# netocg/vae-decode-hdr

Measured on NVIDIA B200. Metric: flux_vae_hdr_decode_megapixels_per_s, higher is better.
Workload: dtype fp16

## Files before the change

vae_decode_hdr_b200/csrc/api.cu:

```cuda
#include <stdarg.h>
#include <string.h>

#include <algorithm>
#include <functional>
#include <map>
#include <string>
#include <vector>

#include "engine.cuh"

namespace hdrvae {

static thread_local std::string g_last_error;
long long g_launch_count = 0;
void set_error(const char* fmt, ...) {
  char buf[1024];
  va_list ap;
  va_start(ap, fmt);
  vsnprintf(buf, sizeof buf, fmt, ap);
  va_end(ap);
  g_last_error = buf;
}

bool g_prof_on = false;
// ... 274 lines not shown
static bool nin_is_fused(hdrvae_ctx* ctx, const ResW& rw, int H, int W) {
  static int on = -1;
  if (on < 0) { const char* e = getenv("HDRVAE_FUSE_NIN"); on = (e && atoi(e) == 0) ? 0 : 1; }
  ConvIO probe;
  return on && rw.has_nin && !ctx->high && rw.nin_x16.w[0] != nullptr && conv_takes_slab(rw.c2, probe, H, W, ctx->conv_impl);
}

static bool x_is_16bit(hdrvae_ctx* ctx) {
  static int on = -1;
  if (on < 0) { const char* e = getenv("HDRVAE_X16"); on = (e && atoi(e) == 0) ? 0 : 1; }
  static int nin_on = -1;
  if (nin_on < 0) { const char* e = getenv("HDRVAE_FUSE_NIN"); nin_on = (e && atoi(e) == 0) ? 0 : 1; }
  return on && nin_on && !ctx->high && ctx->op_dtype == DT_F16 && ctx->conv_impl == HDRVAE_CONV_TCGEN05 && h_is_16bit(ctx);
}

static bool gn_is_fused(hdrvae_ctx* ctx, const PackedConv& pc, const ConvIO& io, int x_dtype, int H, int W) {
  static int on = -1;
  if (on < 0) {
    const char* e = getenv("HDRVAE_FUSE_GN");
    const char* g = getenv("HDRVAE_CTA_GROUP");
    on = ((e && atoi(e) == 0) || (g && atoi(g) == 1)) ? 0 : 1;
  }
  return on && x_is_16bit(ctx) && x_dtype == DT_F16 && pc.w_dtype == DT_F16 && pc.kmul == 1 && !pc.upsample && pc.ks == 3 &&
         pc.cout_pad >= 256 && pc.cin_pad % 64 == 0 && ctx->cta_group != 1 && io.x2 == nullptr && io.y_dtype == DT_F16 &&
         io.stats != nullptr && conv_takes_slab(pc, io, H, W, ctx->conv_impl);
}

static bool attention_fused_enabled(hdrvae_ctx* ctx) {
  static int on = -1;
  if (on < 0) { const char* e = getenv("HDRVAE_ATTN_FUSED"); on = (e && atoi(e) == 0) ? 0 : 1; }
// ... 71 lines not shown
      p.k_per_tap = ks; p.ntaps = 1;
      p.b = v; p.b_row_stride = Tp; p.b_rows = 512; p.n_cols = 512; p.b_img_k_stride = ks;
      p.out = part; p.out_dtype = DT_F32;
      p.out_px_stride = 512; p.out_row_stride = 0; p.out_img_stride = (long long)rows * 512;
      p.sy = p.sx = 1; p.alpha = 1.0f;
      p.tw_log2 = 7; p.TW = 128; p.TH = 1; p.tiles_x = (rows + 127) / 128; p.tiles_y = 1;
      p.cta_group = ctx->cta_group;
      if (impl == HDRVAE_CONV_DIRECT) HDRVAE_TRY(launch_gemm_direct(p, s));
      else HDRVAE_TRY(launch_gemm_tc(p, ctx->num_sms, s));
      HDRVAE_TRY(launch_attn_reduce_splits(part, inv, o_rows, dt, rows, 512, splits, s));
    }
  }
  return 0;
}

static int run_phase_a(hdrvae_ctx* ctx, const void* feat, int B, int H, int W, int pad, float* conv8, void* epi, cudaStream_t s) {
  static int tc_on = -1;
  if (tc_on < 0) { const char* e = getenv("HDRVAE_TC_CONVOUT"); tc_on = (e && atoi(e) == 0) ? 0 : 1; }
  const long long img_stride = (long long)(H + 2 * pad) * W * 128;
  if (ctx->high)
    return launch_epilogue_phase_a(feat, DT_F32, B, H, W, ctx->conv_out_w, ctx->conv_out_b, nullptr, epi, s, 0, img_stride);
  const uint16_t* interior = reinterpret_cast<const uint16_t*>(feat) + (size_t)pad * W * 128;
  if (tc_on && ctx->op_dtype == DT_F16 && ctx->conv_impl == HDRVAE_CONV_TCGEN05 && ctx->conv_out_tc.w[0] != nullptr) {
    ConvIO io; io.x = feat; io.x_pad = pad; io.y = conv8; io.y_dtype = DT_F32; io.y_channels = 8; io.n_store = 8;
    HDRVAE_TRY(run_conv(ctx, ctx->conv_out_tc, io, B, H, W, HDRVAE_CONV_TCGEN05, s));
    return launch_epilogue_phase_a_pre(interior, ctx->op_dtype, B, H, W, conv8, ctx->conv_out_b, nullptr, epi, s, img_stride);
  }
  return launch_epilogue_phase_a(interior, ctx->op_dtype, B, H, W, ctx->conv_out_w, ctx->conv_out_b, nullptr, epi, s, pad, img_stride);
}

static int run_attention_high(hdrvae_ctx* ctx, const Plan& pl, uint8_t* ws, const uint16_t* t3, uint16_t* o3, cudaStream_t s) {
  const int impl = ctx->conv_impl, T = pl.T, Tp = pl.Tp;
  float* f32 = reinterpret_cast<float*>(ws + pl.off_f32);
  uint16_t* q3 = reinterpret_cast<uint16_t*>(ws + pl.off_qk);
  uint16_t* k3 = q3 + (size_t)Tp * 1536;
  uint16_t* vt3 = reinterpret_cast<uint16_t*>(ws + pl.off_vt);
  float* S = reinterpret_cast<float*>(ws + pl.off_s);
  uint16_t* P3 = reinterpret_cast<uint16_t*>(ws + pl.off_p);
// ... 138 lines not shown
  hdrvae_rows* rows;
  cudaStream_t s;
  int B;
  int pad;
  void* lat;
  float* x;
  float* hbuf;
  void* t;
  void* xa16;
  void* xb16;
  void* gn;
  int gn_chunks;
  int* pending;
  int x_dt, h_dt;
  float x_scale, h_scale;
};

static Decoder make_decoder(hdrvae_ctx* ctx, hdrvae_rows* rows, cudaStream_t s, int B, int* pending) {
  Decoder d;
  memset(&d, 0, sizeof d);
  d.ctx = ctx; d.rows = rows; d.s = s; d.B = B; d.pad = rows != nullptr ? 1 : 0; d.pending = pending;
  const bool x16 = x_is_16bit(ctx), h16 = h_is_16bit(ctx);
  d.x_dt = x16 ? ctx->op_dtype : DT_F32; d.x_scale = x16 ? kRawOperandScale : 1.f;
  d.h_dt = h16 ? ctx->op_dtype : DT_F32; d.h_scale = h16 ? kRawOperandScale : 1.f;
  return d;
}

static int step(Decoder& d, std::function<int(cudaStream_t)> fn) {
  if (d.rows == nullptr) return fn(d.s);
  hdrvae_rows::Op op; op.exchange = false; op.fn = std::move(fn); memset(&op.ex, 0, sizeof op.ex);
// ... 117 lines not shown
  ConvIO sc; sc.x = d.xb16; sc.y = d.hbuf; sc.alpha = 1.0f / kRawOperandScale;
  HDRVAE_TRY(conv(d, rw.nin, sc, H, W, kNoStats));
  io.y = d.hbuf; io.residual = d.hbuf;
  HDRVAE_TRY(conv(d, rw.c2, io, H, W));
  std::swap(d.x, d.hbuf);
  return 0;
}

static int decode_to_attention(Decoder& d, int H, int W) {
  ConvIO io; io.x = d.lat; io.y = d.x; io.y_dtype = d.x_dt; io.y_scale = d.x_scale;
  HDRVAE_TRY(conv(d, d.ctx->conv_in, io, H, W, d.x_dt != DT_F32 ? kZeroHalos : 0));
  HDRVAE_TRY(decode_res(d, d.ctx->mid1, H, W));
  return norm(d, d.x, d.x_dt, d.x_scale, d.ctx->attn_norm, false, H, W);
}

static int decode_from_attention(Decoder& d, const void* o, int H, int W) {
  hdrvae_ctx* ctx = d.ctx;
  const bool x16 = d.x_dt != DT_F32;
  {
    ConvIO io; io.x = o; io.y = d.x; io.residual = d.x;
    io.y_dtype = d.x_dt; io.y_scale = d.x_scale; io.res_dtype = d.x_dt; io.res_scale = 1.f / d.x_scale;
    HDRVAE_TRY(conv(d, ctx->proj_out, io, H, W, kDenseInput));
  }
  HDRVAE_TRY(decode_res(d, ctx->mid2, H, W));
  for (int lvl = 3; lvl >= 0; --lvl) {
    for (int i = 0; i < 3; ++i) HDRVAE_TRY(decode_res(d, ctx->up[lvl][i], H, W));
    if (lvl != 0) {
      ConvIO io; io.x = d.xa16; io.y = d.hbuf; io.alpha = 1.0f / kRawOperandScale;
      if (x16) { io.x = d.x; io.y_dtype = d.x_dt; io.y_scale = d.x_scale; }
      else if (lvl <= 2) { io.y2 = d.xb16; io.y2_dtype = ctx->op_dtype; io.y2_scale = kRawOperandScale; }
      HDRVAE_TRY(conv(d, ctx->upsample[lvl], io, H, W, x16 ? kZeroHalos : 0));
      std::swap(d.x, d.hbuf);
      H *= 2; W *= 2;
    }
  }
  return norm(d, d.x, d.x_dt, d.x_scale, ctx->norm_out, true, H, W, ctx->high ? DT_F32 : -1);
}

static int attend_dense(Decoder& d, const Plan& pl, uint8_t* ws, const void** o_out) {
  hdrvae_ctx* ctx = d.ctx;
  const int B = d.B, impl = ctx->conv_impl, dt = ctx->op_dtype;
  cudaStream_t s = d.s;
  void* qk = ws + pl.off_qk;
  void* vt = ws + pl.off_vt;
  void* o = ws + pl.off_o;
  *o_out = o;
  if (ctx->high) {
    ProfScope prof("attention (high precision, GEMM form)", 4.0 * B * (double)pl.T * pl.T * 512 * 3, 0.0, s);
    for (int b = 0; b < B; ++b)
      HDRVAE_TRY(run_attention_high(ctx, pl, ws, reinterpret_cast<const uint16_t*>(d.t) + (size_t)b * pl.T * 1536,
// ... 6 lines not shown
    for (int b = 0; b < B; ++b) {
      const uint16_t* tb = reinterpret_cast<const uint16_t*>(d.t) + (size_t)b * pl.T * 512;
      HDRVAE_TRY(run_gemm(ctx, dt, tb, 512, pl.T, 512, ctx->qk.w[0], 512, 1024, 1024,
                          reinterpret_cast<uint16_t*>(qk) + (size_t)b * pl.Tp * 1024, 1024, dt, ctx->qk.bias, false, 1.0f,
                          nullptr, impl, s));
      HDRVAE_TRY(run_gemm(ctx, dt, ctx->vproj.w[0], 512, 512, 512, tb, 512, pl.T, pl.Tp,
                          reinterpret_cast<uint16_t*>(vt) + (size_t)b * 512 * pl.Tp, pl.Tp, dt, ctx->vproj.bias, true, 1.0f,
                          nullptr, impl, s));
    }
  }
  ProfScope prof("attention core (QK^T, softmax, PV)", 4.0 * B * (double)pl.T * pl.T * 512, 10.0 * B * (double)pl.T * pl.Tp, s);
  return run_attention_core(ctx, pl, ws, qk, vt, o, 1.0f, d.hbuf, (size_t)B * pl.T * 64 * 256 * 4, s);
}

static int run_decoder(hdrvae_ctx* ctx, const float* latent, const Plan& pl, uint8_t* ws, void** features,
                       cudaStream_t s) {
  HDRVAE_REQUIRE(ctx->loaded, "hdrvae: weights not loaded");
  const int B = pl.B, H = pl.h, W = pl.w;
  int pending = 0;
  Decoder d = make_decoder(ctx, nullptr, s, B, &pending);
  d.lat = ws + pl.off_lat;
  d.x = reinterpret_cast<float*>(ws + pl.off_x);
  d.hbuf = reinterpret_cast<float*>(ws + pl.off_h);
  d.t = ws + pl.off_t;
  d.xa16 = ws + pl.off_x16;
  d.xb16 = ws + pl.off_x16b;
  d.gn = ws + pl.off_gn;
  d.gn_chunks = pl.gn_chunks;
  HDRVAE_TRY(gn_scratch_reset(d.gn, B, pl.gn_chunks, s));
  if (ctx->high) {
    float* latf = reinterpret_cast<float*>(ws + pl.off_f32) + (size_t)pl.Tp * 1536;
    HDRVAE_TRY(launch_latent_to_nhwc(latent, latf, DT_F32, B, ctx->c_z, ctx->c_lat, ctx->pq_w, ctx->pq_b, H * W, 64, s));
    HDRVAE_TRY(launch_split3(latf, 64, d.lat, 192, (long long)B * H * W, 64, 1.f, 0, s));
  } else {
    HDRVAE_TRY(launch_latent_to_nhwc(latent, d.lat, ctx->op_dtype, B, ctx->c_z, ctx->c_lat, ctx->pq_w, ctx->pq_b, H * W, 64, s));
  }
  HDRVAE_TRY(decode_to_attention(d, H, W));
  const void* o = nullptr;
  HDRVAE_TRY(attend_dense(d, pl, ws, &o));
  HDRVAE_TRY(decode_from_attention(d, o, H, W));
  *features = d.t;
  return 0;
}

static void attend_rows(Decoder& d, int W, const void** o_out) {
  hdrvae_rows* st = d.rows;
  hdrvae_ctx* ctx = d.ctx;
  const RowsPlan& pl = st->pl;
  uint8_t* ws = st->ws;
  const int rank = st->rank, dt = ctx->op_dtype;
  uint16_t* qk = reinterpret_cast<uint16_t*>(ws + pl.off_qk);
  uint16_t* vb = reinterpret_cast<uint16_t*>(ws + pl.off_v);
  uint16_t* vt = reinterpret_cast<uint16_t*>(ws + pl.off_vt);
  uint16_t* o = reinterpret_cast<uint16_t*>(ws + pl.off_o);
  *o_out = o;
  const uint16_t* tl = reinterpret_cast<const uint16_t*>(d.t) + (size_t)W * 512;
// ... 331 lines not shown
  HDRVAE_CUDA_OK(cudaGraphLaunch(exec, s));
  return 0;
}

int hdrvae_decode_begin(hdrvae_ctx* ctx, const float* latent, int B, int h, int w, void* workspace, size_t ws_bytes,
                        void** raw_stats_dev, void* stream) {
  HDRVAE_REQUIRE(ctx != nullptr && latent != nullptr, "hdrvae_decode: null argument");
  HDRVAE_REQUIRE(B >= 1 && h >= 1 && w >= 1, "hdrvae_decode: empty latent batch [%d,%d,%d,%d]", B, ctx->c_lat, h, w);
  HDRVAE_CUDA_OK(cudaSetDevice(ctx->device));
  const Plan pl = make_plan(B, h, w, false, ctx->high, ctx->high || !attention_fused_enabled(ctx), ctx->c_lat);
  HDRVAE_TRY(check_ws(pl, workspace, ws_bytes));
  uint8_t* ws = reinterpret_cast<uint8_t*>(workspace);
  cudaStream_t s = reinterpret_cast<cudaStream_t>(stream);
  auto body = [&](const float* lat) -> int {
    void* feat = nullptr;
    HDRVAE_TRY(run_decoder(ctx, lat, pl, ws, &feat, s));
    ProfScope prof("epilogue phase A (conv_out, max-pool, stats)", 2.0 * B * 64.0 * h * w * 3 * 1152, B * 64.0 * h * w * (256 + 24), s);
    return run_phase_a(ctx, feat, B, 8 * h, 8 * w, 0, reinterpret_cast<float*>(ws + pl.off_h), ws + pl.off_epi, s);
  };
  if (graphs_enabled(ctx, s)) {
    float* lat_in = reinterpret_cast<float*>(ws + pl.off_lat_in);
    HDRVAE_CUDA_OK(cudaMemcpyAsync(lat_in, latent, (size_t)B * ctx->c_lat * pl.T * 4, cudaMemcpyDeviceToDevice, s));
    hdrvae_ctx::GraphEntry key{0, B, h, w, 0, ctx->conv_impl, ctx->cta_group, 0.f, 0.f, workspace, nullptr, 0};
    HDRVAE_TRY(run_segment(ctx, key, s, [&]() { return body(lat_in); }));
  } else {
    HDRVAE_TRY(body(latent));
  }
  if (raw_stats_dev != nullptr) *raw_stats_dev = epilogue_raw_stats_ptr(ws + pl.off_epi, B, 8 * h, 8 * w);
  return 0;
}

// ... 348 lines not shown
```

vae_decode_hdr_b200/csrc/common.cuh:

```cuda
#pragma once
#include <cuda.h>
#include <cuda_bf16.h>
#include <cuda_fp16.h>
#include <cuda_runtime.h>
#include <stdint.h>
#include <stdio.h>

#include <string>

namespace hdrvae {

void set_error(const char* fmt, ...);
extern long long g_launch_count;
#define HDRVAE_LAUNCHED() (++::hdrvae::g_launch_count)

#define HDRVAE_CUDA_OK(expr)                                                                  \
  do {                                                                                        \
    cudaError_t _e = (expr);                                                                  \
    if (_e != cudaSuccess) {                                                                  \
      ::hdrvae::set_error("%s:%d: %s -> %s", __FILE__, __LINE__, #expr, cudaGetErrorString(_e)); \
      return -1;                                                                              \
    }                                                                                         \
  } while (0)

// ... 118 lines not shown
  const float2 two = make_float2(2.f, 2.f);
  float2 r = make_float2(__int_as_float(0x7EF311C7 - __float_as_int(d.x)), __int_as_float(0x7EF311C7 - __float_as_int(d.y)));
  r = f2_mul(r, f2_fma(nd, r, two));
  r = f2_mul(r, f2_fma(nd, r, two));
  return f2_mul(v, r);
}
__device__ __forceinline__ float silu_nr(float v) {
  float e;
  asm("ex2.approx.ftz.f32 %0, %1;" : "=f"(e) : "f"(fminf(-v * 1.4426950408889634f, 80.f)));
  const float d = 1.f + e;
  float r = __int_as_float(0x7EF311C7 - __float_as_int(d));
  r = r * fmaf(-d, r, 2.f);
  r = r * fmaf(-d, r, 2.f);
  return v * r;
}
#endif

struct PerDeviceOnce {
  bool done[64] = {};
  bool first() {
    int d = 0;
    if (cudaGetDevice(&d) != cudaSuccess || d < 0 || d >= 64) return true;
    if (done[d]) return false;
    done[d] = true;
    return true;
  }
};

struct TensorMapPair {
  CUtensorMap a, b, a2, b2;
// ... 4 lines not shown
```

vae_decode_hdr_b200/csrc/engine.cuh:

```cuda
#pragma once
#include <string>
#include <vector>
#include <map>

#include "../../include/hdrvae.h"
#include "common.cuh"

namespace hdrvae {

int launch_gemm_tc(const GemmParams& p, int num_sms, cudaStream_t stream);
int launch_gemm_direct(const GemmParams& p, cudaStream_t s);
void choose_tile(int H, int W, GemmParams* p);
int launch_to_f32(const void* src, int dtype, float* dst, long long n, cudaStream_t s);
int launch_pack_weight(const float* w, void* out, int out_dtype, int cout, int cin, int ks, int ntaps, int cin_pad,
                       const int* tap_mask, float scale, cudaStream_t s, int split3 = 0);
int launch_add_vectors(const float* a, const float* b, float* c, int n, cudaStream_t s);
int launch_split3(const float* x, long long x_ld, void* out, long long out_ld, long long n, int C, float scale, int order,
                  cudaStream_t s);
int launch_latent_to_nhwc(const float* z, void* out, int out_dtype, int B, int C, int C_lat, const float* pq_w,
                          const float* pq_b, int HW, int cpad, cudaStream_t s);
int launch_latent_rows_to_nhwc(const float* z, void* out, int out_dtype, int C, int C_lat, const float* pq_w,
                               const float* pq_b, int h, int w, int y0, int rows, int cpad, cudaStream_t s);
int launch_softmax_rows(const float* s, void* p, int p_dtype, float* inv_sum, int n_rows, int n_valid, int n_pad,
                        long long s_ld, long long p_ld, cudaStream_t st);
// ... 16 lines not shown
                     float in_scale = 1.f);
size_t epilogue_scratch_bytes(int B, int H, int W);
void* epilogue_raw_stats_ptr(void* scratch, int B, int H, int W);
hdrvae_stats* epilogue_stats_dev_ptr(void* scratch, int B, int H, int W);
float* epilogue_post3_ptr(void* scratch, int B, int H, int W);
float* epilogue_pre3_ptr(void* scratch, int B, int H, int W);
int launch_epilogue_phase_a(const void* pre, int dtype, int B, int H, int W, const float* conv_w, const float* conv_b,
                            int* argmax3, void* scratch, cudaStream_t s, int y_pad = 0, long long img_stride = 0);
double* gn_sums_ptr(void* scratch, int B, int C, int max_chunks);
int launch_gn_reduce_partials(void* scratch, int B, int C, int max_chunks, int n_partials, cudaStream_t s);
int launch_gn_apply_from_sums(const void* x, int x_dtype, long long x_img_stride, void* y, int y_dtype, long long y_img_stride,
                              int B, int rows_px, int C, const float* gamma, const float* beta, bool silu, void* scratch,
                              int max_chunks, double count, cudaStream_t s, float in_scale = 1.f);
int launch_epilogue_phase_a_pre(const void* pre, int dtype, int B, int H, int W, const float* conv8, const float* conv_b,
                                int* argmax3, void* scratch, cudaStream_t s, long long img_stride);
int launch_split_hi_lo(const float* w, float* w8, int k, cudaStream_t s);
int launch_epilogue_phase_b(int B, int H, int W, int mode, float factor, float ev, float* out, hdrvae_stats* host_stats,
                            void* scratch, cudaStream_t s);
int attention_key_splits(int n_keys);
int launch_attention_fused(const void* q, long long q_ld, long long q_img_stride, int n_q, const void* k, long long k_ld,
                           long long k_img_stride, int k_rows, const void* vt, long long vt_ld, long long vt_img_stride,
                           int n_keys, void* o, long long o_img_stride, int n_img, int dt, float alpha, int cta_group,
                           int num_sms, float* part, float* ml, long long part_rows, cudaStream_t s);
int launch_raw_stats_merge(const hdrvae_raw_stats* blocks, int n, hdrvae_raw_stats* dst, cudaStream_t s);

constexpr int kRowsMaxRanks = 16;
struct RowsRawSlot { hdrvae_raw_stats s; unsigned char pad[32]; };
struct RowsMailbox {
  unsigned int arrived[64];
  unsigned int data[64];
// ... 139 lines not shown
```

vae_decode_hdr_b200/csrc/epilogue.cu:

```cuda
#include "../../include/hdrvae.h"
#include "common.cuh"

namespace hdrvae {

constexpr int kTileW = 64, kTileH = 16;
constexpr int kPxPerThread = 4;
constexpr int kHaloW = kTileW + 2, kHaloH = kTileH + 2;
constexpr int kRowPitch = 68;
constexpr int kTilePx = kHaloW * kHaloH;
constexpr int kChanStride = kRowPitch * kHaloH;
constexpr int kChunk = 16;
constexpr int kC = 128;
constexpr int kEpiThreads = (kTileW / kPxPerThread) * kTileH;

struct PartialA {
  float vmin[4];
  float vmax[4];
  double vsum[8];
};

struct PartialB {
  float omin, omax, imax, pad;
  unsigned long long hdr, neg, ihdr, pad2;
};
// ... 37 lines not shown
    const float2 b = __bfloat1622float2(*reinterpret_cast<const __nv_bfloat162*>(&r.y));
    return make_float4(a.x, a.y, b.x, b.y);
  }
};
template <> struct Cvt4<__half> {
  static __device__ __forceinline__ float4 cvt(const uint2& r) {
    const float2 a = __half22float2(*reinterpret_cast<const __half2*>(&r.x));
    const float2 b = __half22float2(*reinterpret_cast<const __half2*>(&r.y));
    return make_float4(a.x, a.y, b.x, b.y);
  }
};

__device__ __forceinline__ float warp_min(float v) { for (int o = 16; o; o >>= 1) v = fminf(v, __shfl_xor_sync(~0u, v, o)); return v; }
__device__ __forceinline__ float warp_max(float v) { for (int o = 16; o; o >>= 1) v = fmaxf(v, __shfl_xor_sync(~0u, v, o)); return v; }
__device__ __forceinline__ double warp_sum(double v) { for (int o = 16; o; o >>= 1) v += __shfl_xor_sync(~0u, v, o); return v; }

template <bool kArgmax>
__device__ __forceinline__ void maxpool_update(float v, int c, float& m, int& idx) {
  if (kArgmax) { if (v > m) { m = v; idx = c; } }
  else m = fmaxf(m, v);
}

template <typename T, bool kArgmax>
__global__ void __launch_bounds__(kEpiThreads, 2)
hdr_phase_a_kernel(const T* __restrict__ pre, const float* __restrict__ conv_w ,
                   const float* __restrict__ conv_b, int H, int W, float* __restrict__ post3,
                   float* __restrict__ pre3, int* __restrict__ argmax3, PartialA* __restrict__ partials, int y_pad,
                   long long img_stride) {
  extern __shared__ float sm[];
  float4* wsm = reinterpret_cast<float4*>(sm);
// ... 125 lines not shown
#pragma unroll
      for (int k = 0; k < 3; ++k) {
        const float cv = acc[q][k] + cb[k];
        const float sv = fminf(fmaxf(__fdiv_rn(__fadd_rn(cv, 1.0f), 2.0f), 0.f), 1.f);
        post3[o + k] = sv;
        pre3[o + k] = mx[q][k];
        if (kArgmax) argmax3[o + k] = am[q][k];
        cmin = fminf(cmin, cv); cmax = fmaxf(cmax, cv); csum += cv;
        pmin = fminf(pmin, sv); pmax = fmaxf(pmax, sv); psum += sv; psq += sv * sv;
        p3min = fminf(p3min, mx[q][k]); p3max = fmaxf(p3max, mx[q][k]);
        hl += mx[q][k] > 1.0f ? 1.f : 0.f;
      }
    }
  }

  __shared__ float rmin[4][8], rmax[4][8];
  __shared__ double rsum[8][8];
  const int warp = tid >> 5, lane = tid & 31;
  const float mins[4] = {warp_min(smin), warp_min(pmin), warp_min(cmin), warp_min(p3min)};
  const float maxs[4] = {warp_max(smax), warp_max(pmax), warp_max(cmax), warp_max(p3max)};
  const double sums[8] = {warp_sum((double)ssum), warp_sum((double)ssq), warp_sum((double)psum), warp_sum((double)psq),
                          warp_sum((double)csum), 0.0, warp_sum((double)nlive), warp_sum((double)hl)};
  if (lane == 0) {
    for (int k = 0; k < 4; ++k) { rmin[k][warp] = mins[k]; rmax[k][warp] = maxs[k]; }
    for (int k = 0; k < 8; ++k) rsum[k][warp] = sums[k];
  }
  __syncthreads();
  if (tid == 0) {
    PartialA pa;
    for (int k = 0; k < 4; ++k) {
      float a = rmin[k][0], b = rmax[k][0];
      for (int w2 = 1; w2 < 8; ++w2) { a = fminf(a, rmin[k][w2]); b = fmaxf(b, rmax[k][w2]); }
      pa.vmin[k] = a; pa.vmax[k] = b;
    }
    for (int k = 0; k < 8; ++k) {
      double a = 0.0;
      for (int w2 = 0; w2 < 8; ++w2) a += rsum[k][w2];
      pa.vsum[k] = a;
    }
    const int ix = min(kTileW, W - x0), iy = min(kTileH, H - y0);
    pa.vsum[5] = (double)ix * iy * kC;
    partials[(blockIdx.z * gridDim.y + blockIdx.y) * gridDim.x + blockIdx.x] = pa;
  }
}

template <typename T, bool kArgmax>
__global__ void __launch_bounds__(kEpiThreads)
hdr_phase_a_pre_kernel(const T* __restrict__ pre, const float4* __restrict__ conv8, const float* __restrict__ conv_b, int H,
                       int W, float* __restrict__ post3, float* __restrict__ pre3, int* __restrict__ argmax3,
                       PartialA* __restrict__ partials, long long img_stride) {
  const int img = blockIdx.z;
  const int x0 = blockIdx.x * kTileW, y0 = blockIdx.y * kTileH;
  const int tid = threadIdx.x, warp = tid >> 5, lane = tid & 31;
  const int sub = lane & 7;
  const int pq = lane >> 3;
  const T* img_base = pre + (long long)img * img_stride;
  const float cb[3] = {conv_b[0], conv_b[1], conv_b[2]};
  float smin = INFINITY, smax = -INFINITY, ssum = 0.f, ssq = 0.f;
// ... 68 lines not shown
      nlive += 3.f;
#pragma unroll
      for (int k = 0; k < 3; ++k) {
        const float cv = cvv[k];
        const float sv = fminf(fmaxf(__fdiv_rn(__fadd_rn(cv, 1.0f), 2.0f), 0.f), 1.f);
        post3[px * 3 + k] = sv;
        pre3[px * 3 + k] = mx[k];
        if (kArgmax) argmax3[px * 3 + k] = am[k];
        cmin = fminf(cmin, cv); cmax = fmaxf(cmax, cv); csum += cv;
        pmin = fminf(pmin, sv); pmax = fmaxf(pmax, sv); psum += sv; psq += sv * sv;
        p3min = fminf(p3min, mx[k]); p3max = fmaxf(p3max, mx[k]);
        hl += mx[k] > 1.0f ? 1.f : 0.f;
      }
    }
  }
  __shared__ float rmin[4][8], rmax[4][8];
  __shared__ double rsum[8][8];
  const float mins[4] = {warp_min(smin), warp_min(pmin), warp_min(cmin), warp_min(p3min)};
  const float maxs[4] = {warp_max(smax), warp_max(pmax), warp_max(cmax), warp_max(p3max)};
  const double sums[8] = {warp_sum((double)ssum), warp_sum((double)ssq), warp_sum((double)psum), warp_sum((double)psq),
                          warp_sum((double)csum), 0.0, warp_sum((double)nlive), warp_sum((double)hl)};
  if (lane == 0) {
    for (int k = 0; k < 4; ++k) { rmin[k][warp] = mins[k]; rmax[k][warp] = maxs[k]; }
    for (int k = 0; k < 8; ++k) rsum[k][warp] = sums[k];
  }
  __syncthreads();
  if (tid == 0) {
    PartialA pa;
    for (int k = 0; k < 4; ++k) {
      float a = rmin[k][0], b = rmax[k][0];
      for (int w2 = 1; w2 < 8; ++w2) { a = fminf(a, rmin[k][w2]); b = fmaxf(b, rmax[k][w2]); }
      pa.vmin[k] = a; pa.vmax[k] = b;
    }
    for (int k = 0; k < 8; ++k) {
      double a = 0.0;
      for (int w2 = 0; w2 < 8; ++w2) a += rsum[k][w2];
      pa.vsum[k] = a;
    }
    const int ix = min(kTileW, W - x0), iy = min(kTileH, H - y0);
    pa.vsum[5] = (double)ix * iy * kC;
    partials[(blockIdx.z * gridDim.y + blockIdx.y) * gridDim.x + blockIdx.x] = pa;
  }
}

__global__ void __launch_bounds__(256)
hdr_reduce_a_kernel(const PartialA* __restrict__ partials, int n, hdrvae_raw_stats* __restrict__ raw) {
  __shared__ float rmin[4][256], rmax[4][256];
  __shared__ double rsum[8][256];
  float mn[4], mx[4];
  double sm[8];
  for (int k = 0; k < 4; ++k) { mn[k] = INFINITY; mx[k] = -INFINITY; }
  for (int k = 0; k < 8; ++k) sm[k] = 0.0;
  for (int i = threadIdx.x; i < n; i += 256) {
    const PartialA pa = partials[i];
    for (int k = 0; k < 4; ++k) { mn[k] = fminf(mn[k], pa.vmin[k]); mx[k] = fmaxf(mx[k], pa.vmax[k]); }
    for (int k = 0; k < 8; ++k) sm[k] += pa.vsum[k];
  }
// ... 183 lines not shown
  st->hdr_pixels = (long long)hdr; st->negative_pixels = (long long)neg; st->intelligent_hdr_pixels = (long long)ihdr;
  st->accepted = (ihdr > 0 || imax > 1.1f) ? 1 : 0;
}

constexpr int kPhaseBBlocks = 148 * 8;

struct EpilogueScratch {
  float* post3; float* pre3; PartialA* pa; PartialB* pb; hdrvae_raw_stats* raw; HdrScalars* sc; hdrvae_stats* st;
};

static int n_blocks_a(int B, int H, int W) { return B * ceil_div(H, kTileH) * ceil_div(W, kTileW); }

size_t epilogue_scratch_bytes(int B, int H, int W) {
  size_t b = 0;
  b += align_up((size_t)B * H * W * 3 * sizeof(float), 256) * 2;
  b += align_up((size_t)n_blocks_a(B, H, W) * sizeof(PartialA), 256);
  b += align_up((size_t)kPhaseBBlocks * sizeof(PartialB), 256);
  b += 256 * 3;
  return b;
}

static EpilogueScratch carve(void* scratch, int B, int H, int W) {
  EpilogueScratch e;
  uint8_t* p = reinterpret_cast<uint8_t*>(scratch);
  const size_t img = align_up((size_t)B * H * W * 3 * sizeof(float), 256);
  e.post3 = reinterpret_cast<float*>(p); p += img;
  e.pre3 = reinterpret_cast<float*>(p); p += img;
  e.pa = reinterpret_cast<PartialA*>(p); p += align_up((size_t)n_blocks_a(B, H, W) * sizeof(PartialA), 256);
  e.pb = reinterpret_cast<PartialB*>(p); p += align_up((size_t)kPhaseBBlocks * sizeof(PartialB), 256);
  e.raw = reinterpret_cast<hdrvae_raw_stats*>(p); p += 256;
  e.sc = reinterpret_cast<HdrScalars*>(p); p += 256;
  e.st = reinterpret_cast<hdrvae_stats*>(p);
  return e;
}

void* epilogue_raw_stats_ptr(void* scratch, int B, int H, int W) { return carve(scratch, B, H, W).raw; }
hdrvae_stats* epilogue_stats_dev_ptr(void* scratch, int B, int H, int W) { return carve(scratch, B, H, W).st; }
float* epilogue_post3_ptr(void* scratch, int B, int H, int W) { return carve(scratch, B, H, W).post3; }
float* epilogue_pre3_ptr(void* scratch, int B, int H, int W) { return carve(scratch, B, H, W).pre3; }

template <typename T>
static void launch_phase_a(const void* pre, const float* conv_w, const float* conv_b, int H, int W, float* post3, float* pre3,
                           int* argmax3, PartialA* pa, dim3 grid, size_t smem, int y_pad, long long img_stride, cudaStream_t s) {
// ... 36 lines not shown
                                int* argmax3, void* scratch, cudaStream_t s, long long img_stride) {
  HDRVAE_REQUIRE(dtype == HDRVAE_F16 || dtype == HDRVAE_BF16, "epilogue (precomputed conv): 16-bit features only");
  if (img_stride == 0) img_stride = (long long)H * W * kC;
  EpilogueScratch e = carve(scratch, B, H, W);
  const dim3 grid(ceil_div(W, kTileW), ceil_div(H, kTileH), B);
  HDRVAE_REQUIRE(grid.y <= 65535 && grid.z <= 65535, "epilogue: image too large for the launch grid");
  const float4* c8 = reinterpret_cast<const float4*>(conv8);
#define HDRVAE_PA_PRE(T, AM) hdr_phase_a_pre_kernel<T, AM><<<grid, kEpiThreads, 0, s>>>(reinterpret_cast<const T*>(pre), c8, conv_b, \
                                                                                       H, W, e.post3, e.pre3, argmax3, e.pa, img_stride)
  if (dtype == HDRVAE_F16) { if (argmax3) HDRVAE_PA_PRE(__half, true); else HDRVAE_PA_PRE(__half, false); }
  else { if (argmax3) HDRVAE_PA_PRE(__nv_bfloat16, true); else HDRVAE_PA_PRE(__nv_bfloat16, false); }
#undef HDRVAE_PA_PRE
  HDRVAE_LAUNCHED();
  HDRVAE_CUDA_OK(cudaGetLastError());
  hdr_reduce_a_kernel<<<1, 256, 0, s>>>(e.pa, n_blocks_a(B, H, W), e.raw);
  HDRVAE_LAUNCHED();
  HDRVAE_CUDA_OK(cudaGetLastError());
  return 0;
}

int launch_epilogue_phase_b(int B, int H, int W, int mode, float factor, float ev, float* out, hdrvae_stats* host_stats,
                            void* scratch, cudaStream_t s) {
  EpilogueScratch e = carve(scratch, B, H, W);
  HDRVAE_REQUIRE(mode >= 0 && mode <= 3, "epilogue: bad mode %d", mode);
  hdr_scalars_kernel<<<1, 32, 0, s>>>(e.raw, e.sc, e.st);
  HDRVAE_LAUNCHED();
  HDRVAE_CUDA_OK(cudaGetLastError());
  const long long n = (long long)B * H * W * 3;
  int blocks = ceil_div(n, 256);
  if (blocks > kPhaseBBlocks) blocks = kPhaseBBlocks;
// ... 41 lines not shown
```

vae_decode_hdr_b200/csrc/groupnorm.cu:

```cuda
#include <type_traits>

#include "common.cuh"

namespace hdrvae {

constexpr int kGroups = 32;
constexpr int kGnThreads = 256;

template <typename T> struct Ld8;
template <> struct Ld8<float> {
  static __device__ __forceinline__ void ld(const float* p, float (&v)[8]) {
    const float4 a = __ldg(reinterpret_cast<const float4*>(p)), b = __ldg(reinterpret_cast<const float4*>(p) + 1);
    v[0] = a.x; v[1] = a.y; v[2] = a.z; v[3] = a.w; v[4] = b.x; v[5] = b.y; v[6] = b.z; v[7] = b.w;
  }
};
template <> struct Ld8<__nv_bfloat16> {
  static __device__ __forceinline__ void ld(const __nv_bfloat16* p, float (&v)[8]) {
    const uint4 r = __ldg(reinterpret_cast<const uint4*>(p));
    const __nv_bfloat162* h = reinterpret_cast<const __nv_bfloat162*>(&r);
#pragma unroll
    for (int e = 0; e < 4; ++e) { const float2 f = __bfloat1622float2(h[e]); v[2 * e] = f.x; v[2 * e + 1] = f.y; }
  }
};
template <> struct Ld8<__half> {
// ... 139 lines not shown
    const int g = c / cpg;
    const double mean = rs[0][g] / count;
    double var = rq[0][g] / count - mean * mean;
    if (var < 0.0) var = 0.0;
    const float rstd = (float)(1.0 / sqrt(var + (double)eps));
    const float a = gamma[c] * rstd;
    scale[(long long)img * C + c] = a;
    shift[(long long)img * C + c] = beta[c] - (float)mean * a;
  }
}
static int gn_slices(int n_chunks) {
  int sl = n_chunks / 32;
  return sl < 1 ? 1 : (sl > kGnSlices ? kGnSlices : sl);
}


template <int kExp> __device__ __forceinline__ float silu_sel(float v) {
  return kExp == 1 ? silu_mufu(v) : kExp == 2 ? silu_nr(v) : silu_f(v);
}

template <bool kSilu, int kExp>
__device__ __forceinline__ void norm_act8(float (&v)[8], const float (&a)[8], const float (&b)[8]) {
#pragma unroll
  for (int j = 0; j < 8; j += 2) {
    float2 t = f2_fma(make_float2(v[j], v[j + 1]), make_float2(a[j], a[j + 1]), make_float2(b[j], b[j + 1]));
    if (kSilu) {
      if (kExp == 2) t = silu_nr2(t);
      else t = make_float2(silu_sel<kExp>(t.x), silu_sel<kExp>(t.y));
    }
    v[j] = t.x; v[j + 1] = t.y;
  }
}

template <typename TIn, typename TOut, bool kSilu, int kMufu = 0>
__global__ void __launch_bounds__(kGnThreads)
gn_apply_kernel(const TIn* __restrict__ x, TOut* __restrict__ y, const float* __restrict__ scale,
                const float* __restrict__ shift, int HW, int C, int px_per_block, long long x_img_stride,
                long long y_img_stride, float in_scale) {
  extern __shared__ float tab[];
  const int img = blockIdx.y;
  for (int c = threadIdx.x; c < C; c += kGnThreads) {
    tab[c] = scale[(long long)img * C + c];
    tab[C + c] = shift[(long long)img * C + c];
  }
  __syncthreads();
  const int vpp = C >> 3;
  const int vi = threadIdx.x % vpp;
// ... 235 lines not shown
```

Baseline: 119.2.

## Fuse norm_out apply with pre-conv_out stats and max-pool in decoder tail

Adds a fused decoder tail. One kernel applies the final GroupNorm+SiLU, writes the fp16 activation, and also computes the pre-conv max-pool and stats. After the tensor-core conv_out, a separate post kernel computes the post-activation stats. Before, the normalized full-resolution 128-channel tensor was written by the GN apply and then re-read by epilogue phase A, so this removes one full pass over it at the cost of another kernel and a larger partials buffer.

```diff
diff --git a/vae_decode_hdr_b200/csrc/api.cu b/vae_decode_hdr_b200/csrc/api.cu
--- a/vae_decode_hdr_b200/csrc/api.cu
+++ b/vae_decode_hdr_b200/csrc/api.cu
@@ -312,6 +312,13 @@
   return on && nin_on && !ctx->high && ctx->op_dtype == DT_F16 && ctx->conv_impl == HDRVAE_CONV_TCGEN05 && h_is_16bit(ctx);
 }
 
+static bool conv_out_on_tc(hdrvae_ctx* ctx);
+static bool tail_is_fused(hdrvae_ctx* ctx) {
+  static int on = -1;
+  if (on < 0) { const char* e = getenv("HDRVAE_FUSED_TAIL"); on = (e && atoi(e) == 0) ? 0 : 1; }
+  return on && x_is_16bit(ctx) && conv_out_on_tc(ctx);
+}
+
 static bool gn_is_fused(hdrvae_ctx* ctx, const PackedConv& pc, const ConvIO& io, int x_dtype, int H, int W) {
   static int on = -1;
   if (on < 0) {
@@ -413,14 +420,18 @@
   return 0;
 }
 
-static int run_phase_a(hdrvae_ctx* ctx, const void* feat, int B, int H, int W, int pad, float* conv8, void* epi, cudaStream_t s) {
+static bool conv_out_on_tc(hdrvae_ctx* ctx) {
   static int tc_on = -1;
   if (tc_on < 0) { const char* e = getenv("HDRVAE_TC_CONVOUT"); tc_on = (e && atoi(e) == 0) ? 0 : 1; }
+  return tc_on && ctx->op_dtype == DT_F16 && ctx->conv_impl == HDRVAE_CONV_TCGEN05 && ctx->conv_out_tc.w[0] != nullptr;
+}
+
+static int run_phase_a(hdrvae_ctx* ctx, const void* feat, int B, int H, int W, int pad, float* conv8, void* epi, cudaStream_t s) {
   const long long img_stride = (long long)(H + 2 * pad) * W * 128;
   if (ctx->high)
     return launch_epilogue_phase_a(feat, DT_F32, B, H, W, ctx->conv_out_w, ctx->conv_out_b, nullptr, epi, s, 0, img_stride);
   const uint16_t* interior = reinterpret_cast<const uint16_t*>(feat) + (size_t)pad * W * 128;
-  if (tc_on && ctx->op_dtype == DT_F16 && ctx->conv_impl == HDRVAE_CONV_TCGEN05 && ctx->conv_out_tc.w[0] != nullptr) {
+  if (conv_out_on_tc(ctx)) {
     ConvIO io; io.x = feat; io.x_pad = pad; io.y = conv8; io.y_dtype = DT_F32; io.y_channels = 8; io.n_store = 8;
     HDRVAE_TRY(run_conv(ctx, ctx->conv_out_tc, io, B, H, W, HDRVAE_CONV_TCGEN05, s));
     return launch_epilogue_phase_a_pre(interior, ctx->op_dtype, B, H, W, conv8, ctx->conv_out_b, nullptr, epi, s, img_stride);
@@ -589,6 +600,7 @@
   int* pending;
   int x_dt, h_dt;
   float x_scale, h_scale;
+  void* epi;
 };
 
 static Decoder make_decoder(hdrvae_ctx* ctx, hdrvae_rows* rows, cudaStream_t s, int B, int* pending) {
@@ -736,6 +748,22 @@
   return norm(d, d.x, d.x_dt, d.x_scale, d.ctx->attn_norm, false, H, W);
 }
 
+static int fused_tail(Decoder& d, int H, int W) {
+  hdrvae_ctx* ctx = d.ctx;
+  const NormW& n = ctx->norm_out;
+  ProfScope prof("epilogue phase A (norm_out, conv_out, max-pool, stats)", 2.0 * d.B * H * W * 3 * 1152,
+                 d.B * (double)H * W * (256 + 256 + 12 + 256 + 32 + 32 + 12), d.s);
+  const int partials = *d.pending;
+  *d.pending = 0;
+  const float *scale = nullptr, *shift = nullptr;
+  HDRVAE_TRY(launch_gn_scale_shift(d.B, H * W, n.C, n.gamma, n.beta, d.gn, d.gn_chunks, partials, d.s, &scale, &shift));
+  HDRVAE_TRY(launch_epilogue_tail_pre(d.x, 1.f / d.x_scale, scale, shift, d.t, d.B, H, W, d.epi, d.s));
+  float* conv8 = d.hbuf;
+  ConvIO io; io.x = d.t; io.y = conv8; io.y_dtype = DT_F32; io.y_channels = 8; io.n_store = 8;
+  HDRVAE_TRY(run_conv(ctx, ctx->conv_out_tc, io, d.B, H, W, HDRVAE_CONV_TCGEN05, d.s));
+  return launch_epilogue_tail_post(conv8, ctx->conv_out_b, d.B, H, W, d.epi, d.s);
+}
+
 static int decode_from_attention(Decoder& d, const void* o, int H, int W) {
   hdrvae_ctx* ctx = d.ctx;
   const bool x16 = d.x_dt != DT_F32;
@@ -756,6 +784,7 @@
       H *= 2; W *= 2;
     }
   }
+  if (d.epi != nullptr) return fused_tail(d, H, W);
   return norm(d, d.x, d.x_dt, d.x_scale, ctx->norm_out, true, H, W, ctx->high ? DT_F32 : -1);
 }
 
@@ -792,7 +821,7 @@
 }
 
 static int run_decoder(hdrvae_ctx* ctx, const float* latent, const Plan& pl, uint8_t* ws, void** features,
-                       cudaStream_t s) {
+                       cudaStream_t s, void* epi = nullptr) {
   HDRVAE_REQUIRE(ctx->loaded, "hdrvae: weights not loaded");
   const int B = pl.B, H = pl.h, W = pl.w;
   int pending = 0;
@@ -805,6 +834,7 @@
   d.xb16 = ws + pl.off_x16b;
   d.gn = ws + pl.off_gn;
   d.gn_chunks = pl.gn_chunks;
+  if (epi != nullptr && tail_is_fused(ctx)) d.epi = epi;
   HDRVAE_TRY(gn_scratch_reset(d.gn, B, pl.gn_chunks, s));
   if (ctx->high) {
     float* latf = reinterpret_cast<float*>(ws + pl.off_f32) + (size_t)pl.Tp * 1536;
@@ -817,7 +847,7 @@
   const void* o = nullptr;
   HDRVAE_TRY(attend_dense(d, pl, ws, &o));
   HDRVAE_TRY(decode_from_attention(d, o, H, W));
-  *features = d.t;
+  *features = d.epi != nullptr ? nullptr : d.t;
   return 0;
 }
 
@@ -1179,7 +1209,8 @@
   cudaStream_t s = reinterpret_cast<cudaStream_t>(stream);
   auto body = [&](const float* lat) -> int {
     void* feat = nullptr;
-    HDRVAE_TRY(run_decoder(ctx, lat, pl, ws, &feat, s));
+    HDRVAE_TRY(run_decoder(ctx, lat, pl, ws, &feat, s, ws + pl.off_epi));
+    if (feat == nullptr) return 0;
     ProfScope prof("epilogue phase A (conv_out, max-pool, stats)", 2.0 * B * 64.0 * h * w * 3 * 1152, B * 64.0 * h * w * (256 + 24), s);
     return run_phase_a(ctx, feat, B, 8 * h, 8 * w, 0, reinterpret_cast<float*>(ws + pl.off_h), ws + pl.off_epi, s);
   };
diff --git a/vae_decode_hdr_b200/csrc/common.cuh b/vae_decode_hdr_b200/csrc/common.cuh
--- a/vae_decode_hdr_b200/csrc/common.cuh
+++ b/vae_decode_hdr_b200/csrc/common.cuh
@@ -156,6 +156,22 @@
   r = r * fmaf(-d, r, 2.f);
   return v * r;
 }
+template <int kExp> __device__ __forceinline__ float silu_sel(float v) {
+  return kExp == 1 ? silu_mufu(v) : kExp == 2 ? silu_nr(v) : silu_f(v);
+}
+
+template <bool kSilu, int kExp>
+__device__ __forceinline__ void norm_act8(float (&v)[8], const float (&a)[8], const float (&b)[8]) {
+#pragma unroll
+  for (int j = 0; j < 8; j += 2) {
+    float2 t = f2_fma(make_float2(v[j], v[j + 1]), make_float2(a[j], a[j + 1]), make_float2(b[j], b[j + 1]));
+    if (kSilu) {
+      if (kExp == 2) t = silu_nr2(t);
+      else t = make_float2(silu_sel<kExp>(t.x), silu_sel<kExp>(t.y));
+    }
+    v[j] = t.x; v[j + 1] = t.y;
+  }
+}
 #endif
 
 struct PerDeviceOnce {
diff --git a/vae_decode_hdr_b200/csrc/engine.cuh b/vae_decode_hdr_b200/csrc/engine.cuh
--- a/vae_decode_hdr_b200/csrc/engine.cuh
+++ b/vae_decode_hdr_b200/csrc/engine.cuh
@@ -54,6 +54,9 @@
                               int max_chunks, double count, cudaStream_t s, float in_scale = 1.f);
 int launch_epilogue_phase_a_pre(const void* pre, int dtype, int B, int H, int W, const float* conv8, const float* conv_b,
                                 int* argmax3, void* scratch, cudaStream_t s, long long img_stride);
+int launch_epilogue_tail_pre(const void* x, float in_scale, const float* scale, const float* shift, void* t, int B, int H, int W,
+                             void* scratch, cudaStream_t s);
+int launch_epilogue_tail_post(const float* conv8, const float* conv_b, int B, int H, int W, void* scratch, cudaStream_t s);
 int launch_split_hi_lo(const float* w, float* w8, int k, cudaStream_t s);
 int launch_epilogue_phase_b(int B, int H, int W, int mode, float factor, float ev, float* out, hdrvae_stats* host_stats,
                             void* scratch, cudaStream_t s);
diff --git a/vae_decode_hdr_b200/csrc/epilogue.cu b/vae_decode_hdr_b200/csrc/epilogue.cu
--- a/vae_decode_hdr_b200/csrc/epilogue.cu
+++ b/vae_decode_hdr_b200/csrc/epilogue.cu
@@ -75,6 +75,37 @@
 __device__ __forceinline__ float warp_min(float v) { for (int o = 16; o; o >>= 1) v = fminf(v, __shfl_xor_sync(~0u, v, o)); return v; }
 __device__ __forceinline__ float warp_max(float v) { for (int o = 16; o; o >>= 1) v = fmaxf(v, __shfl_xor_sync(~0u, v, o)); return v; }
 __device__ __forceinline__ double warp_sum(double v) { for (int o = 16; o; o >>= 1) v += __shfl_xor_sync(~0u, v, o); return v; }
+
+__device__ __forceinline__ void write_partial_a(const float (&mn)[4], const float (&mx)[4], const float (&sm)[8], double owned,
+                                                PartialA* __restrict__ dst) {
+  __shared__ float rmin[4][8], rmax[4][8];
+  __shared__ double rsum[8][8];
+  const int warp = threadIdx.x >> 5, lane = threadIdx.x & 31;
+  const float mins[4] = {warp_min(mn[0]), warp_min(mn[1]), warp_min(mn[2]), warp_min(mn[3])};
+  const float maxs[4] = {warp_max(mx[0]), warp_max(mx[1]), warp_max(mx[2]), warp_max(mx[3])};
+  const double sums[8] = {warp_sum((double)sm[0]), warp_sum((double)sm[1]), warp_sum((double)sm[2]), warp_sum((double)sm[3]),
+                          warp_sum((double)sm[4]), 0.0, warp_sum((double)sm[6]), warp_sum((double)sm[7])};
+  if (lane == 0) {
+    for (int k = 0; k < 4; ++k) { rmin[k][warp] = mins[k]; rmax[k][warp] = maxs[k]; }
+    for (int k = 0; k < 8; ++k) rsum[k][warp] = sums[k];
+  }
+  __syncthreads();
+  if (threadIdx.x == 0) {
+    PartialA pa;
+    for (int k = 0; k < 4; ++k) {
+      float a = rmin[k][0], b = rmax[k][0];
+      for (int w2 = 1; w2 < 8; ++w2) { a = fminf(a, rmin[k][w2]); b = fmaxf(b, rmax[k][w2]); }
+      pa.vmin[k] = a; pa.vmax[k] = b;
+    }
+    for (int k = 0; k < 8; ++k) {
+      double a = 0.0;
+      for (int w2 = 0; w2 < 8; ++w2) a += rsum[k][w2];
+      pa.vsum[k] = a;
+    }
+    pa.vsum[5] = owned;
+    *dst = pa;
+  }
+}
 
 template <bool kArgmax>
 __device__ __forceinline__ void maxpool_update(float v, int c, float& m, int& idx) {
@@ -230,34 +261,9 @@
     }
   }
 
-  __shared__ float rmin[4][8], rmax[4][8];
-  __shared__ double rsum[8][8];
-  const int warp = tid >> 5, lane = tid & 31;
-  const float mins[4] = {warp_min(smin), warp_min(pmin), warp_min(cmin), warp_min(p3min)};
-  const float maxs[4] = {warp_max(smax), warp_max(pmax), warp_max(cmax), warp_max(p3max)};
-  const double sums[8] = {warp_sum((double)ssum), warp_sum((double)ssq), warp_sum((double)psum), warp_sum((double)psq),
-                          warp_sum((double)csum), 0.0, warp_sum((double)nlive), warp_sum((double)hl)};
-  if (lane == 0) {
-    for (int k = 0; k < 4; ++k) { rmin[k][warp] = mins[k]; rmax[k][warp] = maxs[k]; }
-    for (int k = 0; k < 8; ++k) rsum[k][warp] = sums[k];
-  }
-  __syncthreads();
-  if (tid == 0) {
-    PartialA pa;
-    for (int k = 0; k < 4; ++k) {
-      float a = rmin[k][0], b = rmax[k][0];
-      for (int w2 = 1; w2 < 8; ++w2) { a = fminf(a, rmin[k][w2]); b = fmaxf(b, rmax[k][w2]); }
-      pa.vmin[k] = a; pa.vmax[k] = b;
-    }
-    for (int k = 0; k < 8; ++k) {
-      double a = 0.0;
-      for (int w2 = 0; w2 < 8; ++w2) a += rsum[k][w2];
-      pa.vsum[k] = a;
-    }
-    const int ix = min(kTileW, W - x0), iy = min(kTileH, H - y0);
-    pa.vsum[5] = (double)ix * iy * kC;
-    partials[(blockIdx.z * gridDim.y + blockIdx.y) * gridDim.x + blockIdx.x] = pa;
-  }
+  const int ix = min(kTileW, W - x0), iy = min(kTileH, H - y0);
+  write_partial_a({smin, pmin, cmin, p3min}, {smax, pmax, cmax, p3max}, {ssum, ssq, psum, psq, csum, 0.f, nlive, hl},
+                  (double)ix * iy * kC, partials + (blockIdx.z * gridDim.y + blockIdx.y) * gridDim.x + blockIdx.x);
 }
 
 template <typename T, bool kArgmax>
@@ -356,33 +362,112 @@
       }
     }
   }
-  __shared__ float rmin[4][8], rmax[4][8];
-  __shared__ double rsum[8][8];
-  const float mins[4] = {warp_min(smin), warp_min(pmin), warp_min(cmin), warp_min(p3min)};
-  const float maxs[4] = {warp_max(smax), warp_max(pmax), warp_max(cmax), warp_max(p3max)};
-  const double sums[8] = {warp_sum((double)ssum), warp_sum((double)ssq), warp_sum((double)psum), warp_sum((double)psq),
-                          warp_sum((double)csum), 0.0, warp_sum((double)nlive), warp_sum((double)hl)};
-  if (lane == 0) {
-    for (int k = 0; k < 4; ++k) { rmin[k][warp] = mins[k]; rmax[k][warp] = maxs[k]; }
-    for (int k = 0; k < 8; ++k) rsum[k][warp] = sums[k];
-  }
-  __syncthreads();
-  if (tid == 0) {
-    PartialA pa;
-    for (int k = 0; k < 4; ++k) {
-      float a = rmin[k][0], b = rmax[k][0];
-      for (int w2 = 1; w2 < 8; ++w2) { a = fminf(a, rmin[k][w2]); b = fmaxf(b, rmax[k][w2]); }
-      pa.vmin[k] = a; pa.vmax[k] = b;
-    }
-    for (int k = 0; k < 8; ++k) {
-      double a = 0.0;
-      for (int w2 = 0; w2 < 8; ++w2) a += rsum[k][w2];
-      pa.vsum[k] = a;
-    }
-    const int ix = min(kTileW, W - x0), iy = min(kTileH, H - y0);
-    pa.vsum[5] = (double)ix * iy * kC;
-    partials[(blockIdx.z * gridDim.y + blockIdx.y) * gridDim.x + blockIdx.x] = pa;
-  }
+  const int ix = min(kTileW, W - x0), iy = min(kTileH, H - y0);
+  write_partial_a({smin, pmin, cmin, p3min}, {smax, pmax, cmax, p3max}, {ssum, ssq, psum, psq, csum, 0.f, nlive, hl},
+                  (double)ix * iy * kC, partials + (blockIdx.z * gridDim.y + blockIdx.y) * gridDim.x + blockIdx.x);
+}
+
+__global__ void __launch_bounds__(kEpiThreads, 3)
+hdr_tail_pre_kernel(const __half* __restrict__ x, float in_scale, const float* __restrict__ scale, const float* __restrict__ shift,
+                    __half* __restrict__ t, int H, int W, float* __restrict__ pre3, PartialA* __restrict__ partials) {
+  const int img = blockIdx.z;
+  const int x0 = blockIdx.x * kTileW, y0 = blockIdx.y * kTileH;
+  const int tid = threadIdx.x;
+  const int vi = tid & 15;
+  const int slot = tid >> 4;
+  float a[8], b[8];
+#pragma unroll
+  for (int j = 0; j < 8; ++j) {
+    a[j] = scale[img * kC + vi * 8 + j] * in_scale;
+    b[j] = shift[img * kC + vi * 8 + j];
+  }
+  const long long img_off = (long long)img * H * W * kC + vi * 8;
+  float smin = INFINITY, smax = -INFINITY, ssum = 0.f, ssq = 0.f;
+  float p3min = INFINITY, p3max = -INFINITY;
+  float hl = 0.f;
+  constexpr int U = 4, kSteps = kTileW * kTileH / (16 * U);
+#pragma unroll 1
+  for (int st = 0; st < kSteps; ++st) {
+    uint4 r[U];
+    long long off[U];
+    bool live[U];
+#pragma unroll
+    for (int u = 0; u < U; ++u) {
+      const int bp = slot + 16 * (st * U + u);
+      const int gx = x0 + (bp % kTileW), gy = y0 + (bp / kTileW);
+      live[u] = gx < W && gy < H;
+      off[u] = img_off + ((long long)gy * W + gx) * kC;
+      r[u] = live[u] ? __ldg(reinterpret_cast<const uint4*>(x + off[u])) : make_uint4(0u, 0u, 0u, 0u);
+    }
+#pragma unroll
+    for (int u = 0; u < U; ++u) {
+      float v[8];
+      const __half2* hp = reinterpret_cast<const __half2*>(&r[u]);
+#pragma unroll
+      for (int e = 0; e < 4; ++e) { const float2 f = __half22float2(hp[e]); v[2 * e] = f.x; v[2 * e + 1] = f.y; }
+      norm_act8<true, 2>(v, a, b);
+      uint4 o;
+      uint32_t* ow = reinterpret_cast<uint32_t*>(&o);
+#pragma unroll
+      for (int e = 0; e < 4; ++e) {
+        const __half2 q = __floats2half2_rn(v[2 * e], v[2 * e + 1]);
+        ow[e] = *reinterpret_cast<const uint32_t*>(&q);
+        const float2 f = __half22float2(q);
+        v[2 * e] = f.x; v[2 * e + 1] = f.y;
+      }
+      if (live[u]) *reinterpret_cast<uint4*>(t + off[u]) = o;
+      float mx[3] = {-INFINITY, -INFINITY, -INFINITY};
+#pragma unroll
+      for (int j = 0; j < 8; ++j) {
+        const int c = vi * 8 + j;
+        if (live[u]) { smin = fminf(smin, v[j]); smax = fmaxf(smax, v[j]); ssum += v[j]; ssq = fmaf(v[j], v[j], ssq); }
+        if (c < 42) mx[0] = fmaxf(mx[0], v[j]);
+        else if (c < 84) mx[1] = fmaxf(mx[1], v[j]);
+        else if (c < 126) mx[2] = fmaxf(mx[2], v[j]);
+      }
+#pragma unroll
+      for (int o2 = 1; o2 < 16; o2 <<= 1)
+#pragma unroll
+        for (int k = 0; k < 3; ++k) mx[k] = fmaxf(mx[k], __shfl_xor_sync(~0u, mx[k], o2));
+      if (live[u] && vi == 0) {
+        const long long px = off[u] / kC;
+#pragma unroll
+        for (int k = 0; k < 3; ++k) {
+          pre3[px * 3 + k] = mx[k];
+          p3min = fminf(p3min, mx[k]); p3max = fmaxf(p3max, mx[k]);
+          hl += mx[k] > 1.0f ? 1.f : 0.f;
+        }
+      }
+    }
+  }
+  const int ix = min(kTileW, W - x0), iy = min(kTileH, H - y0);
+  write_partial_a({smin, INFINITY, INFINITY, p3min}, {smax, -INFINITY, -INFINITY, p3max}, {ssum, ssq, 0.f, 0.f, 0.f, 0.f, 0.f, hl},
+                  (double)ix * iy * kC, partials + (blockIdx.z * gridDim.y + blockIdx.y) * gridDim.x + blockIdx.x);
+}
+
+constexpr int kPostBlocks = 148 * 4;
+__global__ void __launch_bounds__(kEpiThreads)
+hdr_post_kernel(const float4* __restrict__ conv8, const float* __restrict__ conv_b, long long n_px, float* __restrict__ post3,
+                PartialA* __restrict__ partials) {
+  const float cb[3] = {conv_b[0], conv_b[1], conv_b[2]};
+  float cmin = INFINITY, cmax = -INFINITY, csum = 0.f;
+  float pmin = INFINITY, pmax = -INFINITY, psum = 0.f, psq = 0.f;
+  float nlive = 0.f;
+  for (long long px = blockIdx.x * (long long)kEpiThreads + threadIdx.x; px < n_px; px += (long long)gridDim.x * kEpiThreads) {
+    const float4 hi = conv8[px * 2], lo = conv8[px * 2 + 1];
+    const float cvv[3] = {(hi.x + lo.x) + cb[0], (hi.y + lo.y) + cb[1], (hi.z + lo.z) + cb[2]};
+    nlive += 3.f;
+#pragma unroll
+    for (int k = 0; k < 3; ++k) {
+      const float cv = cvv[k];
+      const float sv = fminf(fmaxf(__fdiv_rn(__fadd_rn(cv, 1.0f), 2.0f), 0.f), 1.f);
+      post3[px * 3 + k] = sv;
+      cmin = fminf(cmin, cv); cmax = fmaxf(cmax, cv); csum += cv;
+      pmin = fminf(pmin, sv); pmax = fmaxf(pmax, sv); psum += sv; psq += sv * sv;
+    }
+  }
+  write_partial_a({INFINITY, pmin, cmin, INFINITY}, {-INFINITY, pmax, cmax, -INFINITY}, {0.f, 0.f, psum, psq, csum, 0.f, nlive, 0.f},
+                  0.0, partials + blockIdx.x);
 }
 
 __global__ void __launch_bounds__(256)
@@ -596,7 +681,7 @@
 size_t epilogue_scratch_bytes(int B, int H, int W) {
   size_t b = 0;
   b += align_up((size_t)B * H * W * 3 * sizeof(float), 256) * 2;
-  b += align_up((size_t)n_blocks_a(B, H, W) * sizeof(PartialA), 256);
+  b += align_up((size_t)(n_blocks_a(B, H, W) + kPostBlocks) * sizeof(PartialA), 256);
   b += align_up((size_t)kPhaseBBlocks * sizeof(PartialB), 256);
   b += 256 * 3;
   return b;
@@ -608,7 +693,7 @@
   const size_t img = align_up((size_t)B * H * W * 3 * sizeof(float), 256);
   e.post3 = reinterpret_cast<float*>(p); p += img;
   e.pre3 = reinterpret_cast<float*>(p); p += img;
-  e.pa = reinterpret_cast<PartialA*>(p); p += align_up((size_t)n_blocks_a(B, H, W) * sizeof(PartialA), 256);
+  e.pa = reinterpret_cast<PartialA*>(p); p += align_up((size_t)(n_blocks_a(B, H, W) + kPostBlocks) * sizeof(PartialA), 256);
   e.pb = reinterpret_cast<PartialB*>(p); p += align_up((size_t)kPhaseBBlocks * sizeof(PartialB), 256);
   e.raw = reinterpret_cast<hdrvae_raw_stats*>(p); p += 256;
   e.sc = reinterpret_cast<HdrScalars*>(p); p += 256;
@@ -675,6 +760,33 @@
   HDRVAE_LAUNCHED();
   HDRVAE_CUDA_OK(cudaGetLastError());
   hdr_reduce_a_kernel<<<1, 256, 0, s>>>(e.pa, n_blocks_a(B, H, W), e.raw);
+  HDRVAE_LAUNCHED();
+  HDRVAE_CUDA_OK(cudaGetLastError());
+  return 0;
+}
+
+int launch_epilogue_tail_pre(const void* x, float in_scale, const float* scale, const float* shift, void* t, int B, int H, int W,
+                             void* scratch, cudaStream_t s) {
+  EpilogueScratch e = carve(scratch, B, H, W);
+  const dim3 grid(ceil_div(W, kTileW), ceil_div(H, kTileH), B);
+  HDRVAE_REQUIRE(grid.y <= 65535 && grid.z <= 65535, "epilogue: image too large for the launch grid");
+  hdr_tail_pre_kernel<<<grid, kEpiThreads, 0, s>>>(reinterpret_cast<const __half*>(x), in_scale, scale, shift,
+                                                   reinterpret_cast<__half*>(t), H, W, e.pre3, e.pa);
+  HDRVAE_LAUNCHED();
+  HDRVAE_CUDA_OK(cudaGetLastError());
+  return 0;
+}
+
+int launch_epilogue_tail_post(const float* conv8, const float* conv_b, int B, int H, int W, void* scratch, cudaStream_t s) {
+  EpilogueScratch e = carve(scratch, B, H, W);
+  const long long n_px = (long long)B * H * W;
+  int blocks = ceil_div(n_px, kEpiThreads);
+  if (blocks > kPostBlocks) blocks = kPostBlocks;
+  const int n_pre = n_blocks_a(B, H, W);
+  hdr_post_kernel<<<blocks, kEpiThreads, 0, s>>>(reinterpret_cast<const float4*>(conv8), conv_b, n_px, e.post3, e.pa + n_pre);
+  HDRVAE_LAUNCHED();
+  HDRVAE_CUDA_OK(cudaGetLastError());
+  hdr_reduce_a_kernel<<<1, 256, 0, s>>>(e.pa, n_pre + blocks, e.raw);
   HDRVAE_LAUNCHED();
   HDRVAE_CUDA_OK(cudaGetLastError());
   return 0;
diff --git a/vae_decode_hdr_b200/csrc/groupnorm.cu b/vae_decode_hdr_b200/csrc/groupnorm.cu
--- a/vae_decode_hdr_b200/csrc/groupnorm.cu
+++ b/vae_decode_hdr_b200/csrc/groupnorm.cu
@@ -177,23 +177,6 @@
   return sl < 1 ? 1 : (sl > kGnSlices ? kGnSlices : sl);
 }
 
-
-template <int kExp> __device__ __forceinline__ float silu_sel(float v) {
-  return kExp == 1 ? silu_mufu(v) : kExp == 2 ? silu_nr(v) : silu_f(v);
-}
-
-template <bool kSilu, int kExp>
-__device__ __forceinline__ void norm_act8(float (&v)[8], const float (&a)[8], const float (&b)[8]) {
-#pragma unroll
-  for (int j = 0; j < 8; j += 2) {
-    float2 t = f2_fma(make_float2(v[j], v[j + 1]), make_float2(a[j], a[j + 1]), make_float2(b[j], b[j + 1]));
-    if (kSilu) {
-      if (kExp == 2) t = silu_nr2(t);
-      else t = make_float2(silu_sel<kExp>(t.x), silu_sel<kExp>(t.y));
-    }
-    v[j] = t.x; v[j + 1] = t.y;
-  }
-}
 
 template <typename TIn, typename TOut, bool kSilu, int kMufu = 0>
 __global__ void __launch_bounds__(kGnThreads)
```

New measurement: 119.5 (median of 6 runs). About the same (+0.2%).
